# hidasib/GRU4Rec

Hardware: AMD Instinct MI355X
Metric: mini-batches/sec (gru4rec.py:661), RSC15-shaped batch=128 n_sample=2048 BPR-max (higher is better)
Workload: dtype f32

## Files before the change

gru4rec_amd/csrc/g4r_host_create.hpp:

```cpp

int g4r_device_count(void) {
    int n = 0;
    if (hipGetDeviceCount(&n) != hipSuccess) return 0;
    return n;
}
const char* g4r_last_error(void) { return g_err.c_str(); }
#ifndef G4R_HIPCC_VERSION
#define G4R_HIPCC_VERSION "unknown"
#endif
const char* g4r_version(void) { return "gru4rec_hip 0.4 (gfx950; hipcc " G4R_HIPCC_VERSION "; isa-audited)"; }
int g4r_sizeof_config(void) { return (int)sizeof(g4r_config); }

static int build_lean_args(g4r_model* m) {
    DevModel& d = m->dm;
    const StepKernels& k = m->kern;
    const int L = d.n_layers;
    std::vector<LeanV> av(L); std::vector<LeanH> ah(L); std::vector<LeanDa> aa(L); std::vector<LeanDy> ay(L);
    const bool constrained = d.embed_mode == G4R_EMBED_CONSTRAINED;
    bool any_layer = false;
    for (int l = 0; l < L; ++l) {
        if (k.fwd[l] != FWD_LEAN) continue;
        any_layer = true;
        LeanV& v = av[l]; memset(&v, 0, sizeof(v));
        v.Wx = d.dense_p + d.offWx[l]; v.Wrz = d.dense_p + d.offWrz[l]; v.Bh = d.dense_p + d.offBh[l];
// ... 56 lines not shown
        const size_t nslot = cdiv((long long)d.R * 16 * sizeof(int), (long long)sizeof(DenseTile));
        if (dalloc(m, &m->d_tiles16, tiles.size() + nslot) || dalloc(m, &m->d_leanU, (size_t)1)) return -1;
        d.own_pos = m->sw.owner_scan_in_update ? nullptr : (int*)(m->d_tiles16 + tiles.size());
        m->h_leanU.own_on = d.own_pos ? 1 : 0;
        HIPCHK(hipMemcpyAsync(m->d_tiles16, tiles.data(), tiles.size() * sizeof(DenseTile), hipMemcpyHostToDevice, m->stream));
        HIPCHK(hipStreamSynchronize(m->stream));
    }
    HIPCHK(hipStreamSynchronize(m->stream));
    return 0;
}

static KernelSwitches read_switches(const g4r_config& cfg) {
    KernelSwitches w;
    w.no_lean = getenv("G4R_NO_LEAN") != nullptr; w.no_mt = getenv("G4R_NO_MT") != nullptr; w.no_bmt = getenv("G4R_NO_BMT") != nullptr;
    w.no_merge = getenv("G4R_NO_MERGE") != nullptr; w.owner_scan_in_update = env_int("G4R_OWNER_SCAN", 0) != 0;
    w.allow_lean_update = env_int("G4R_LEAN_UPDATE", 1) != 0; w.defer = env_int("G4R_DEFER", cfg.defer_updates) != 0;
    w.p2_geo = env_int("G4R_P2_GEO", -1); w.ba_geo = env_int("G4R_BA_GEO", -1);
    w.wide2 = env_int("G4R_WIDE2", -1); w.p1_ks = env_int("G4R_P1_KS", 128); w.bb_ks = env_int("G4R_BB_KS", 0);
    const char* skip = getenv("G4R_SKIP_KN");
    w.skip_kn = skip ? strtoull(skip, nullptr, 0) : 0ull;
    return w;
}

int g4r_create(const g4r_config* cfg, g4r_model** out) {
    if (!cfg || !out) return fail("null argument");
    if (cfg->n_layers < 1 || cfg->n_layers > G4R_MAX_LAYERS) return fail("n_layers out of range");
    if (cfg->batch_size < 1 || cfg->n_items < 1) return fail("batch_size / n_items must be positive");
    for (int l = 0; l < cfg->n_layers; ++l)
        if (cfg->layers[l] % 4 != 0 || cfg->layers[l] < 4 || cfg->layers[l] > 1024)
            return fail("layer sizes must be multiples of 4 in [4, 1024]");
// ... 259 lines not shown
```

gru4rec_amd/csrc/g4r_host_debug.hpp:

```cpp
int g4r_get_debug(g4r_model* m, const char* name, float* host, int64_t count) {
    if (!m || !name || !host) return fail("null argument");
    HIPCHK(hipSetDevice(m->cfg.device));
    DevModel& d = m->dm;
    const StepKernels& k = m->kern;
    std::string s(name);
    const float* p = nullptr; int64_t n = 0;
    int l = 0;
    if (!s.empty() && isdigit((unsigned char)s.back())) { l = s.back() - '0'; s.pop_back(); }
    if (l >= d.n_layers) return fail("layer out of range");
    const int64_t bd = (int64_t)d.B * d.D[l];
    if (s == "scores") { p = d.Sc; n = (int64_t)d.B * d.ldSc; }
    else if (s == "dSx") { p = d.dSx + (size_t)((m->gstep - 1) & d.defer_mask) * (size_t)d.dSx_stride; n = (int64_t)d.B * d.Ein; }
    else if (s == "dSy") { p = d.dSy + (size_t)((m->gstep - 1) & d.defer_mask) * (size_t)d.dSy_stride; n = (int64_t)d.ldSc * d.Dtop; }
    else if (s == "dSBy") { p = d.dSBy + (size_t)((m->gstep - 1) & d.defer_mask) * (size_t)d.dSBy_stride; n = d.ldSc; }
    else if (s == "defer_stats") {
        if (count < 4) return fail("count");
        double rows = 0, bias = 0;
        if (m->defer_on) {
            std::vector<unsigned> st(2048);
            HIPCHK(hipStreamSynchronize(m->stream));
            HIPCHK(hipMemcpy(st.data(), d.dstat, st.size() * sizeof(unsigned), hipMemcpyDeviceToHost));
            for (size_t i = 0; i < st.size(); i += 2) { rows += st[i]; bias += st[i + 1]; }
        }
        host[0] = (float)rows; host[1] = (float)bias; host[2] = m->defer_on ? 1.f : 0.f; host[3] = (float)(d.defer_mask + 1);
// ... 36 lines not shown
        for (int l = 0; l < d.n_layers; ++l) mk |= k.fwd[l] == FWD_LEAN ? 1 << l : 0;
        host[0] = (float)mk; host[1] = k.score_fwd == SF_LEAN ? 1.f : 0.f; host[2] = k.score_bwd == SB_LEAN ? 1.f : 0.f;
        host[3] = k.update == UP_LEAN ? 1.f : 0.f;
        return 0;
    }
    else if (s == "kernels") {
        const int ML = G4R_MAX_LAYERS;
        const int tail[] = {k.score_fwd, k.loss_spec, k.loss_long, k.loss_quads, k.score_bwd, k.kch, k.ksplit, k.bmt_slabs, k.update, k.chunks, k.wide_dense, k.finish_rows};
        if (count < 4 * ML + 12) return fail("count");
        for (int i = 0; i < 4 * ML + 12; ++i) host[i] = i < 4 * ML ? 0.f : (float)tail[i - 4 * ML];
        for (int l = 0; l < d.n_layers; ++l) {
            host[l] = (float)k.fwd[l]; host[ML + l] = (float)k.bwd[l]; host[2 * ML + l] = (float)(k.p2_deep[l] + 2 * k.ba_deep[l]); host[3 * ML + l] = (float)k.wg[l].use;
        }
        return 0;
    }
    else if (s == "n_cu") { if (count < 1) return fail("count"); host[0] = (float)m->n_cu; return 0; }
    else if (s == "ksplit") { if (count < 1) return fail("count"); host[0] = (float)d.ksplit; return 0; }
    else if (s == "dev_syncs") { if (count < 1) return fail("count"); host[0] = (float)m->n_dev_syncs; return 0; }
    else if (s == "dense_count") { if (count < 1) return fail("count"); host[0] = (float)d.dense_count; return 0; }
    else if (s == "occ_score_tile") {
        if (count < 1) return fail("count");
        int nb = 0;
        for (size_t lds = SMEM_SF2; lds >= SMEM_SF2 - 2048; lds -= 512) {
            HIPCHK(hipOccupancyMaxActiveBlocksPerMultiprocessor(&nb, (const void*)k_score_fwd_t2, GT_NTH, lds));
            fprintf(stderr, "[g4r] k_score_fwd_t2 dynamic LDS %zu -> %d workgroups per CU\n", lds, nb);
        }
        host[0] = (float)nb;
        return 0;
    }
    else if (s == "graph_mode") {
// ... 132 lines not shown
```

gru4rec_amd/csrc/g4r_host_model.hpp:

```cpp
static thread_local std::string g_err;
static int fail(const std::string& s) { g_err = s; return -1; }
void g4r_set_error(const char* fmt, ...) {
    char buf[1024];
    va_list ap;
    va_start(ap, fmt);
    vsnprintf(buf, sizeof(buf), fmt, ap);
    va_end(ap);
    g_err = buf;
}
#define HIPCHK(x)                                                                                        \
    do {                                                                                                 \
        hipError_t e_ = (x);                                                                             \
        if (e_ != hipSuccess)                                                                            \
            return fail(std::string(#x) + ": " + hipGetErrorString(e_) + " @" + std::to_string(__LINE__)); \
    } while (0)
#define NCCLCHK(x)                                                                                         \
    do {                                                                                                   \
        ncclResult_t e_ = (x);                                                                             \
        if (e_ != ncclSuccess)                                                                             \
            return fail(std::string(#x) + ": " + ncclGetErrorString(e_) + " @" + std::to_string(__LINE__)); \
    } while (0)

enum { KN_GRU_P1 = 0, KN_GRU_P2, KN_SCORE_FWD, KN_LOSS, KN_SCORE_BWD, KN_BWD_PRE, KN_BWD_A, KN_BWD_B, KN_DENSE, KN_ALLREDUCE,
       KN_DENSE_APPLY, KN_SPARSE, KN_UPDATE, KN_BWD_FUSED, KN_FWD_FUSED, KN_GATE, KN_FLUSH, KN_SCAN, KN_FINISH, KN_GRU_V, KN_GRU_H, KN_GRU_DA, KN_GRU_DY, KN_COUNT };
static const char* KN_NAMES[KN_COUNT] = {"k_gru_p1", "k_gru_p2", "k_score_fwd", "k_loss_rows", "k_score_bwd", "k_gru_bwd_pre",
                                         "k_gru_bwd_a", "k_gru_bwd_b", "k_dense_grad", "rccl_allreduce", "k_dense_apply",
                                         "k_sparse_update", "k_update", "k_gru_bwd", "k_gru_fwd", "k_gru_gate", "k_sparse_flush", "k_defer_scan", "k_finish_rows", "k_gru_v", "k_gru_h", "k_gru_da", "k_gru_dy"};

struct EvRec { int kn; hipEvent_t a, b; };

struct KernelSwitches {
    bool no_lean = false;
    bool no_mt = false, no_bmt = false;
    bool no_merge = false;
    bool allow_lean_update = true;
    bool owner_scan_in_update = false;
    bool defer = false;
    int p2_geo = -1, ba_geo = -1;
    int wide2 = -1, p1_ks = 128, bb_ks = 0;
    unsigned long long skip_kn = 0;
};
enum GruFwdKind { FWD_LEAN = 0 , FWD_FUSED = 1 , FWD_P1S = 2 ,
                  FWD_P1_N64 = 3, FWD_P1_N32 = 4 };
enum GruBwdKind { BWD_LEAN = 0 , BWD_FUSED = 1 , BWD_ONEHOT = 2, BWD_BW = 3, BWD_B = 4 };
enum ScoreFwdKind { SF_LEAN = 0 , SF_MT = 1 , SF_T3 = 2, SF_T2 = 3, SF_K64 = 4, SF_K128 = 5  };
enum ScoreBwdKind { SB_LEAN = 0 , SB_BMT = 1 , SB_BWD2 = 2 , SB_W = 3, SB_N = 4  };
enum UpdateKind { UP_LEAN = 0 , UP_MERGED = 1 , UP_SPLIT = 2 };
struct WideGeo { int use = 0, ny = 1, nh = 1, kys = 0, khs = 0, bbn = 1, bbk = 0; };
struct StepKernels {
    int fwd[G4R_MAX_LAYERS], bwd[G4R_MAX_LAYERS];
    int p2_deep[G4R_MAX_LAYERS], ba_deep[G4R_MAX_LAYERS];
    WideGeo wg[G4R_MAX_LAYERS];
    int score_fwd;
    int loss_spec, loss_long, loss_quads;
    int score_bwd;
    int kch, ksplit;
    int bmt_slabs;
    int nblkA, nblkB, ndtA, ndtB, nrtB;
    int update;
    int chunks;
    int wide_dense;
    int finish_rows;
};

struct g4r_model {
    g4r_config cfg;
    DevModel dm;
    DevModel* d_dm = nullptr;
    int n_cu = 256;
    KernelSwitches sw;
// ... 234 lines not shown
    const bool lean_s = !sw.no_lean && Dt <= LN_MAXD && Dt % 4 == 0 && !wide && !dma && B < 65536 && d.ldSc < 65536;
    k.score_fwd = lean_s ? SF_LEAN : mt ? SF_MT : dma ? SF_T3 : (wide && Dt % T2_BK == 0) ? SF_T2 : wide ? SF_K64 : SF_K128;
    k.loss_spec = (d.final_act == G4R_ACT_ELU && d.loss == G4R_LOSS_BPR_MAX) ? 1 : (d.final_act == G4R_ACT_SOFTMAX && d.loss == G4R_LOSS_XE) ? 2
                : (d.final_act == G4R_ACT_ELU && d.loss == G4R_LOSS_TOP1_MAX) ? 3 : 0;
    k.loss_long = (size_t)(2 * d.ldSc + 18 * LOSS_NW) * sizeof(float) > (size_t)(156 * 1024);
    k.loss_quads = d.ldSc >= 4 * LOSS_T;
    const bool bwd2 = wide && Dt % 64 == 0;
    const bool top_tiles = k.bwd[top] != BWD_LEAN && k.bwd[top] != BWD_FUSED;
    if (!sw.no_bmt && bwd2 && top_tiles && Dt % 128 == 0 && Dt <= 512 && d.ldSc % BMT_WA == 0 && d.ldSc <= 0xFFFF && B <= 0xFFFF) {
        const int ntA = d.ldSc / BMT_WA * (Dt / 32), den = cdiv(B, 64) * (Dt / 128), ks = ntA / den;
        if (ntA % den == 0 && ntA % 8 == 0 && ntA <= n_cu && ntA * 8 >= n_cu * 7 && BMT_WA % (Dt / 32) == 0 && 4 * (BMT_WA / (Dt / 32)) <= 256 &&
            ks >= 2 && ks <= 24 && d.ldSc % ks == 0 && (d.ldSc / ks) % 32 == 0 && d.ldSc / ks <= 2048)
            k.bmt_slabs = ks;
    }
    k.score_bwd = (lean_s && B <= 128) ? SB_LEAN : k.bmt_slabs ? SB_BMT : bwd2 ? SB_BWD2 : wide ? SB_W : SB_N;
    const int slabs_target = top_tiles ? 17 : 9;
    k.kch = GT_BK * std::max(1, (cdiv(d.ldSc, GT_BK) + slabs_target / 2) / slabs_target);
    if (k.score_bwd == SB_LEAN) k.kch = 128;
    else if (k.score_bwd == SB_BMT) k.kch = d.ldSc / k.bmt_slabs;
    else if (k.score_bwd == SB_BWD2) {
        const int ndt = Dt / 64, nrt = cdiv(B, 64), nA = cdiv(d.ldSc, 64) * ndt;
        double best = 2.0;
        for (int ks = 12; ks <= 24; ++ks) {
            const int kch = (cdiv(d.ldSc, ks) + 7) & ~7;
            if (cdiv(d.ldSc, kch) != ks) continue;
            const double rounds = (double)(nA + ks * nrt * ndt) / n_cu;
            const double waste = (std::ceil(rounds) - rounds) / std::ceil(rounds) + 1e-3 * std::abs(ks - 17);
            if (waste < best) { best = waste; k.kch = kch; }
        }
    }
// ... 20 lines not shown
```

gru4rec_amd/csrc/g4r_host_step.hpp:

```cpp
static int launch_step(g4r_model* m, std::vector<EvRec>* recs, int part = 0) {
    DevModel& d = m->dm;
    const StepKernels& k = m->kern;
    const int L = d.n_layers, B = d.B;
    hipStream_t s = m->stream;
    GruFwdPredict nopa = {};
    size_t evi = 0;
    hipEvent_t cur_a = nullptr, cur_b = nullptr;
    static const bool trace = getenv("G4R_TRACE") != nullptr;
    int trace_kn = -1;
    auto begin = [&](int kn) {
        trace_kn = kn;
        if (trace) { fprintf(stderr, "[g4r] launch %s\n", KN_NAMES[kn]); fflush(stderr); }
        if (!recs) return;
        while (m->evs.size() < evi + 2) { hipEvent_t e; (void)hipEventCreate(&e); m->evs.push_back(e); }
        EvRec r = {kn, m->evs[evi], m->evs[evi + 1]};
        evi += 2;
        cur_a = r.a; cur_b = r.b;
        recs->push_back(r);
    };
    auto end = [&]() {
        if (trace) {
            hipError_t e = hipStreamSynchronize(s);
            fprintf(stderr, "[g4r] done   %s: %s\n", KN_NAMES[trace_kn], hipGetErrorString(e));
            fflush(stderr);
        }
    };
#define LK(kern, grid, block, smem, strm, ...)                                                             \
    do {                                                                                                  \
        if (m->sw.skip_kn && trace_kn >= 0 && ((m->sw.skip_kn >> trace_kn) & 1ull)) break;                \
        if (recs) hipExtLaunchKernelGGL(kern, grid, block, smem, strm, cur_a, cur_b, 0, __VA_ARGS__);     \
        else hipLaunchKernelGGL(kern, grid, block, smem, strm, __VA_ARGS__);                              \
    } while (0)
    const DevModel* dmp = (const DevModel*)m->d_dm;
    StepState* stp = (StepState*)d.st;
    const bool merged = k.update != UP_SPLIT && !(recs && m->profile_split);
    if (part != 2) {
    for (int l = 0; l < L; ++l) {
        if (k.fwd[l] == FWD_LEAN) {
            const int ntd = cdiv(d.D[l], 16), nrb = cdiv(B, 16);
            begin(KN_GRU_V);
            {
                const LeanV& v = m->h_leanV[l];
                const unsigned dims = (unsigned)d.D[l] | ((unsigned)d.IN[l] << 16);
#define G4R_LK_V(L0_, DR_) LK((k_gru_v<L0_, DR_>), dim3(ntd, nrb, 3), dim3(512), 0, s, (const LeanV*)(m->d_leanV + l), (StepState*)v.st, (const int*)v.cur_in, \
                              (const float*)v.Wx, (const float*)v.Wrz, (const float*)v.H0, (const float*)v.H1, dims, (unsigned)B)
                if (l > 0) G4R_LK_V(false, false); else if (d.drop_e > 0.f) G4R_LK_V(true, true); else G4R_LK_V(true, false);
#undef G4R_LK_V
            }
            end();
            begin(KN_GRU_H);
// ... 58 lines not shown
        do {                                                                                                                   \
            if (k.loss_spec == 1) LK((k_loss_rows<L, 1, V>), gloss, dim3(LOSS_T), m->smem_loss, s, dmp, stp);        \
            else if (k.loss_spec == 2) LK((k_loss_rows<L, 2, V>), gloss, dim3(LOSS_T), m->smem_loss, s, dmp, stp);   \
            else if (k.loss_spec == 3) LK((k_loss_rows<L, 3, V>), gloss, dim3(LOSS_T), m->smem_loss, s, dmp, stp);   \
            else LK((k_loss_rows<L, 0, V>), gloss, dim3(LOSS_T), m->smem_loss, s, dmp, stp);                         \
        } while (0)
        if (k.loss_long) G4R_LK_LOSS(true, 4);
        else { if (k.loss_quads) G4R_LK_LOSS(false, 4); else G4R_LK_LOSS(false, 1); }
#undef G4R_LK_LOSS
    }
    end();
    begin(KN_SCORE_BWD);
    switch (k.score_bwd) {
    case SB_LEAN: {
        const LeanB& q = m->h_leanB;
        LK(k_score_b, dim3(q.nA + d.ksplit * q.nrb * q.ndb), dim3(512), 0, s, (const LeanB*)m->d_leanB, (const int*)(d.cur_in + 2 * B), (const int*)d.cur_col,
           (const float*)d.Sc, (const float*)d.hd[L - 1], (const float*)d.Wy, (float*)d.accWy, (unsigned)d.Dtop | ((unsigned)B << 16), (unsigned)d.N | ((unsigned)d.ldSc << 16));
        break;
    }
    case SB_BMT: {
        const int ntile = d.ldSc / BMT_WA * (d.Dtop / 32);
        LK(k_score_bmt, dim3(2 * ntile), dim3(256), SMEM_BMT, s, (const float*)d.Sc, (const float*)d.hd[L - 1], (const float*)d.Wy, (const int*)d.col_item,
           (const int*)(d.cur_in + 2 * B), (const float*)d.zrow, dmp, (unsigned)d.Dtop | ((unsigned)(d.Dtop / 32) << 16), (unsigned)d.N | ((unsigned)d.ldSc << 16),
           (unsigned)B | ((unsigned)d.kch << 16), (unsigned)cdiv(B, 64) | ((unsigned)(d.Dtop / 128) << 16));
        break;
    }
    case SB_BWD2: {
        const int ndt = d.Dtop / 64, nrt = cdiv(B, 64);
        int nA = cdiv(d.ldSc, 64) * ndt, nB = d.ksplit * nrt * ndt, nC = cdiv(d.ldSc, 64);
        LK(k_score_bwd2, dim3(nA + nB + nC), dim3(GT_NTH), (size_t)(4 * 64 * 16) * sizeof(float) + (size_t)std::max(d.kch, 64) * sizeof(int), s, dmp, stp, nA, nB, ndt, nrt);
        break;
    }
// ... 2 lines not shown
    }
    end();
    for (int l = L - 1; l >= 0; --l) {
        if (k.bwd[l] == BWD_LEAN) {
            const int nrb = cdiv(B, 16);
            begin(KN_GRU_DA);
            {
                const LeanDa& q = m->h_leanDa[l];
                LK(k_gru_da, dim3(cdiv(d.D[l], 16), nrb), dim3(128), 0, s, (const LeanDa*)(m->d_leanDa + l), (const int*)(d.cur_in + 2 * B), (const float*)q.dsrc,
                   (const float*)q.Wh, (const float*)q.z, (const float*)q.c, (const float*)q.H0, (const float*)q.H1, (unsigned)d.D[l] | ((unsigned)q.ks << 16), (unsigned)B);
            }
            end();
            begin(KN_GRU_DY);
            {
                const LeanDy& y = m->h_leanDy[l];
                LK(k_gru_dy, dim3(cdiv(d.IN[l], 16), nrb), dim3(1024), 0, s, (const LeanDy*)(m->d_leanDy + l), (const int*)(d.cur_in + 2 * B), (const int*)y.occ_idx,
                   (const float*)y.dV, (const float*)y.drp, (const float*)y.Wx, (const float*)y.r, (unsigned)d.D[l] | ((unsigned)d.IN[l] << 16), (unsigned)B);
            }
            end();
            continue;
        }
        if (k.bwd[l] == BWD_FUSED) {
            begin(KN_BWD_FUSED);
            LK(k_gru_bwd_fused, dim3(cdiv(d.IN[l], 32), cdiv(B, BF_ROWS)), dim3(512), smem_bwd_fused(d.D[l]), s, dmp, stp, l);
            end();
            continue;
        }
        begin(KN_BWD_PRE);
        LK(k_gru_bwd_pre, dim3(cdiv((long long)B * d.D[l], 256)), dim3(256), 0, s, dmp, stp, l);
        end();
// ... 438 lines not shown
```

gru4rec_amd/csrc/g4r_lean_kernels.cuh:

```cuda
#pragma once

#define LN_MAXD 128

__device__ __forceinline__ float ldu(const GAS float* base, unsigned boff) { return *(const GAS float*)((const GAS char*)base + boff); }
__device__ __forceinline__ int ldu_i(const GAS int* base, unsigned boff) { return *(const GAS int*)((const GAS char*)base + boff); }
__device__ __forceinline__ float4 ldu4(const GAS float* base, unsigned boff) { return *(const GAS float4*)((const GAS char*)base + boff); }
__device__ __forceinline__ void stu(GAS float* base, unsigned boff, float v) { *(GAS float*)((GAS char*)base + boff) = v; }
__device__ __forceinline__ void stu4(GAS float* base, unsigned boff, float4 v) { *(GAS float4*)((GAS char*)base + boff) = v; }

#if defined(G4R_CLK_TRACE)
#define LCLK_INIT(dbgp, slot) GAS long long* clk_ = ((dbgp) && blockIdx.x == 1 && blockIdx.y == 1 && blockIdx.z == 0 && threadIdx.x == 0) ? (dbgp) + (slot) : nullptr
#define LCLK(i) do { if (clk_) clk_[i] = wall_clock64(); } while (0)
#define LCLK_USE(x) do { if (clk_ && (x) == 123.456f) clk_[15] = 0; } while (0)
#define LSPAN_BEGIN(tilep, base) GAS long long* span_ = ((tilep) && threadIdx.x == 0) ? (tilep) + 8 * (size_t)((base) + (blockIdx.z * gridDim.y + blockIdx.y) * gridDim.x + blockIdx.x) : nullptr; \
    if (span_) span_[0] = wall_clock64()
#define LSPAN_END() do { if (span_) span_[1] = wall_clock64(); } while (0)
#else
#define LCLK_INIT(dbgp, slot)
#define LCLK(i)
#define LCLK_USE(x)
#define LSPAN_BEGIN(tilep, base)
#define LSPAN_END()
#endif

struct LeanV {
    GP(const float) Wx; GP(const float) Wrz; GP(const float) Bh; GP(const float) H0; GP(const float) H1;
    GP(const float) ysrc;
    GP(const int) cur_in;
    GP(float) Vc; GP(float) r; GP(float) Hr; GP(float) z; GP(float) yin0;
    GP(int) occ_idx; GP(int) occ_fl;
    GP(StepState) st;
    unsigned long long seed;
    int B, D, IN, R, first, pub_fl;
    float drop_e;
    int n_items;
    GP(long long) dbg; GP(long long) dbgtile;
};
// ... 334 lines not shown
    for (int q = 0; q < 4; ++q) acc[q] = mfma16(bq[q].w, da[3], acc[q]);
    LCLK_USE(acc[0][0]); LCLK(5);
    if ((int)row < M) {
        const unsigned ob = j * ps + 4 * (row * D + 4 * lg);
#pragma unroll
        for (int q = 0; q < 4; ++q) {
            const unsigned n = 16 * (4 * wid + q) + 4 * lg;
            if (n < D) stu4(a.drp, ob + 64 * (4 * wid + q), make_float4(acc[q][0], acc[q][1], acc[q][2], acc[q][3]));
        }
    }
    LCLK(6);
    LSPAN_END();
}

#define LN_PL 8
__global__ __launch_bounds__(1024) void k_gru_dy(const LeanDy* __restrict__ ap, const int* meta_, const int* occ_idx_, const float* dV_, const float* drp_,
                                                 const float* Wx_, const float* r_, unsigned dims, unsigned B) {
    __shared__ float sJ[4 * 16 * 64];
    const unsigned tid = threadIdx.x, lane = tid & 63, li = lane & 15, lg = lane >> 4;
    const unsigned wid = __builtin_amdgcn_readfirstlane(tid >> 6);
    const unsigned D = dims & 0xFFFFu, IN = dims >> 16, Dq = D >> 2;
    const unsigned m0 = blockIdx.y * 16, row = m0 + li, rowB = min(row, B - 1);
    const unsigned ncol = 16 * blockIdx.x + li, nc = min(ncol, IN - 1);
    const unsigned rowe = m0 + 4 * lg + (wid & 3);
    const GAS float* Wx = (const GAS float*)Wx_;
#if defined(G4R_CLK_TRACE)
    const long long tk0 = wall_clock64();
    GAS long long* ck = nullptr;
#define DYCK(i) do { if (ck) ck[i] = wall_clock64(); } while (0)
#else
#define DYCK(i)
#endif
    f32x4 acc;
// ... 82 lines not shown
        acc1 = mfma16(s.w, b0.w, acc1);
        acc = acc0 + acc1;
#if defined(G4R_CLK_TRACE)
        if (ck) { if (acc[0] == 123.4f) ck[7] = 0; ck[3] = wall_clock64(); }
#endif
    }
    const int M = sx.M;
    if ((int)m0 >= M) return;
#pragma unroll
    for (int rg = 0; rg < 4; ++rg) sJ[(rg * 16 + wid) * 64 + lane] = acc[rg];
    __syncthreads();
    if (wid >= 4) return;
    const LeanDy a = *ap;
    LCLK_INIT(a.dbg, 48); LCLK(6);
    LSPAN_BEGIN(a.dbgtile, 1500);
    float v = 0.f;
#pragma unroll
    for (int w = 0; w < 16; ++w) v += sJ[(wid * 16 + w) * 64 + lane];
    if (ncol >= IN || (int)rowe >= M) return;
    const unsigned o = 4 * (rowe * IN + ncol);
    if (a.layer0) {
        if (a.drop_e > 0.f) v *= drop_mult(a.seed, sx.g, G4R_STREAM_DROP_EMBED, rowe, ncol, 1.0f - a.drop_e);
        const float an = a2 + G4R_MUT_ACC(v * v);
        GAS float* dSx = a.dSx + (size_t)(sx.g & (unsigned)a.defer_mask) * (size_t)a.dSx_stride;
        stu(dSx, o, a.generic ? v : G4R_MUT_STEP(a.lr * v * frsq(an + G4R_EPS_ADAGRAD)));
        if (!a.generic && cnt2 == 1 && itm >= 0) a.accT[(size_t)itm * IN + ncol] = an;
        else stu(a.dAx, o, an);
    } else {
        stu(a.dylo, o, v);
    }
    LCLK(7);
    LSPAN_END();
}

template <bool LOGQ>
__global__ __launch_bounds__(256) void k_score_s(const LeanS* __restrict__ ap, const int* meta_, const int* cur_col_, const float* hd_, const float* Wy_,
                                                 const float* By_, float* Sc_, unsigned dimsA, unsigned dimsB) {
    __shared__ f32x4 sJ[4 * 4 * 64];
    const unsigned tid = threadIdx.x, lane = tid & 63, li = lane & 15, lg = lane >> 4;
    const unsigned wid = __builtin_amdgcn_readfirstlane(tid >> 6);
    const unsigned D = dimsA & 0xFFFFu, B = dimsA >> 16, N = dimsB & 0xFFFFu, ldSc = dimsB >> 16, Dq = D >> 2;
    const unsigned n0 = blockIdx.x * 32, m0 = blockIdx.y * 32;
    const GAS int* cur_col = (const GAS int*)cur_col_;
    const unsigned nA = n0 + li, nB = n0 + 16 + li;
    int it0 = ldu_i(cur_col, 4 * min(nA, ldSc - 1)), it1 = ldu_i(cur_col, 4 * min(nB, ldSc - 1));
    const int4 mt = ldi4((const GAS int*)meta_);
    const unsigned Q0 = 8 * wid + lg, Q1 = Q0 + 4;
// ... 65 lines not shown
    if (ne >= N) return;
    const unsigned r0 = m0 + 16 * (wid >> 1) + 4 * lg;
    GAS float* Sc = (GAS float*)Sc_;
    float o[4];
#pragma unroll
    for (int rg = 0; rg < 4; ++rg) { o[rg] = v[rg] + bias; lean_keep(o[rg]); }
#pragma unroll
    for (int rg = 0; rg < 4; ++rg)
        if ((int)(r0 + rg) < M) stu(Sc, 4 * ((r0 + rg) * ldSc + ne), o[rg]);
    LCLK(5);
    LSPAN_END();
}
template __global__ void k_score_s<false>(const LeanS*, const int*, const int*, const float*, const float*, const float*, float*, unsigned, unsigned);
template __global__ void k_score_s<true>(const LeanS*, const int*, const int*, const float*, const float*, const float*, float*, unsigned, unsigned);

__global__ __launch_bounds__(512) void k_score_b(const LeanB* __restrict__ ap, const int* meta_, const int* cur_col_, const float* Sc_, const float* hd_,
                                                 const float* Wy_, float* accWy_, unsigned dimsA, unsigned dimsB) {
    __shared__ f32x4 sJ[4 * 8 * 64];
    const unsigned tid = threadIdx.x, lane = tid & 63, li = lane & 15, lg = lane >> 4;
    const unsigned wid = __builtin_amdgcn_readfirstlane(tid >> 6);
    const unsigned D = dimsA & 0xFFFFu, B = dimsA >> 16, N = dimsB & 0xFFFFu, ldSc = dimsB >> 16;
    const GAS int* cur_col = (const GAS int*)cur_col_;
    const GAS float *Sc = (const GAS float*)Sc_, *hd = (const GAS float*)hd_;
    const int4 mt = ldi4((const GAS int*)meta_);
    const LeanB a = *ap;
    LSPAN_BEGIN(a.dbgtile, 2048);
    f32x4 acc[4];
#pragma unroll
    for (int c = 0; c < 4; ++c) acc[c] = (f32x4){0.f, 0.f, 0.f, 0.f};
    if (blockIdx.x < (unsigned)a.nA) {
        const unsigned nt = blockIdx.x / (unsigned)a.ndh, dh_ = blockIdx.x - nt * (unsigned)a.ndh;
        const unsigned n0 = 16 * nt, d0 = 64 * dh_;
        const unsigned n = n0 + li, nc = min(n, ldSc - 1);
        const unsigned d4 = d0 + 16 * lg + 4 * (wid & 3);
        const int item = ldu_i(cur_col, 4 * nc);
        float4 av[4];
        float bv[4];
        const unsigned da = d0 + 4 * li;
        const unsigned dac = min(da, D - 4);
#pragma unroll
        for (int s_ = 0; s_ < 4; ++s_) {
            const unsigned b = min(16 * wid + 4 * s_ + lg, B - 1);
            av[s_] = ldu4(hd, 4 * (b * D + dac));
            bv[s_] = ldu(Sc, 4 * (b * ldSc + nc));
        }
        lean_pin(a.accBy, a.occ_fl);
        const bool iok = item >= 0 && n < N;
        const unsigned ic = (unsigned)max(item, 0);
        float4 acc4 = ld4((const GAS float*)accWy_ + (size_t)ic * D + min(d4, D - 4));
        const float accb = a.accBy[ic];
        const int cnt = a.occ_fl[4 * (size_t)ic + 2];
        if (d4 >= D) acc4 = make_float4(accb, 0.f, 0.f, 0.f);
        __builtin_amdgcn_sched_barrier(0);
        const LeanState sx = lean_state(mt);
        const int M = sx.M;
#pragma unroll
        for (int s_ = 0; s_ < 4; ++s_) {
            const unsigned b = 16 * wid + 4 * s_ + lg;
            const bool bok = (int)b < M;
            float4 h4 = av[s_];
            const float hx[4] = {h4.x, h4.y, h4.z, h4.w};
            float hv[4];
#pragma unroll
            for (int c = 0; c < 4; ++c) hv[c] = (da + c < D) ? hx[c] : ((da + c == D) ? 1.f : 0.f);
            const float dsv = (bok && n < ldSc) ? bv[s_] : 0.f;
#pragma unroll
            for (int c = 0; c < 4; ++c) acc[c] = mfma16(hv[c], dsv, acc[c]);
        }
#pragma unroll
        for (int rg = 0; rg < 4; ++rg) sJ[(rg * 8 + wid) * 64 + lane] = (f32x4){acc[0][rg], acc[1][rg], acc[2][rg], acc[3][rg]};
        __syncthreads();
        if (wid >= 4) return;
        f32x4 g4 = sJ[(wid * 8 + 0) * 64 + lane];
#pragma unroll
        for (int w = 1; w < 8; ++w) g4 += sJ[(wid * 8 + w) * 64 + lane];
        if (n >= N || d4 > D) return;
        const float gg[4] = {g4[0], g4[1], g4[2], g4[3]}, a0[4] = {acc4.x, acc4.y, acc4.z, acc4.w};
        float st[4], an[4];
        const bool generic = a.generic != 0;
#pragma unroll
        for (int c = 0; c < 4; ++c) {
            an[c] = a0[c] + G4R_MUT_ACC(gg[c] * gg[c]);
            st[c] = iok ? G4R_MUT_ROW(n, G4R_MUT_STEP(a.lr * gg[c] * frsq(an[c] + G4R_EPS_ADAGRAD))) : 0.f;
            if (generic) st[c] = iok ? gg[c] : 0.f;
        }
        const bool single = !generic && iok && cnt == 1;
        const size_t slot = (size_t)(sx.g & (unsigned)a.defer_mask);
        if (d4 < D) {
            st4(a.dSy + slot * (size_t)a.dSy_stride + (size_t)n * D + d4, make_float4(st[0], st[1], st[2], st[3]));
            if (single) st4((GAS float*)accWy_ + (size_t)ic * D + d4, make_float4(an[0], an[1], an[2], an[3]));
            else st4(a.dAy + (size_t)n * D + d4, make_float4(an[0], an[1], an[2], an[3]));
        } else {
            (a.dSBy + slot * (size_t)a.dSBy_stride)[n] = st[0];
            if (single) a.accBy[ic] = an[0]; else a.dABy[n] = an[0];
        }
        LSPAN_END();
        return;
    }
    {
        const unsigned w_ = blockIdx.x - (unsigned)a.nA;
        const unsigned per = (unsigned)(a.nrb * a.ndb);
        const unsigned kc = w_ / per, rem = w_ - kc * per, rb = rem / (unsigned)a.ndb, db = rem - rb * (unsigned)a.ndb;
        const unsigned b0 = 16 * rb, d0 = 64 * db;
        const unsigned nk = 128 * kc + 16 * wid + 4 * lg;
        const unsigned nkc = min(nk, ldSc - 4);
        const int4 it4 = ldi4(cur_col + nkc);
        float4 ds4 = ldu4(Sc, 4 * (min(b0 + li, B - 1) * ldSc + nkc));
        const unsigned dq = d0 + 4 * li, dqc = min(dq, D - 4);
        const GAS float* Wy = (const GAS float*)Wy_;
        const int its[4] = {it4.x, it4.y, it4.z, it4.w};
        float4 wv[4];
#pragma unroll
        for (int u = 0; u < 4; ++u) wv[u] = ld4(Wy + (size_t)max(its[u], 0) * D + dqc);
        __builtin_amdgcn_sched_barrier(0);
        const LeanState sx = lean_state(mt);
        const int M = sx.M;
        if ((int)b0 >= M) return;
        const float dsx[4] = {ds4.x, ds4.y, ds4.z, ds4.w};
        const bool bok = (int)(b0 + li) < M;
#pragma unroll
        for (int u = 0; u < 4; ++u) {
            const bool kok = nk + u < ldSc && nk == nkc && its[u] >= 0 && dq < D;
            const float av_ = bok ? dsx[u] : 0.f;
            const float4 w4 = kok ? wv[u] : make_float4(0.f, 0.f, 0.f, 0.f);
            acc[0] = mfma16(av_, w4.x, acc[0]);
            acc[1] = mfma16(av_, w4.y, acc[1]);
            acc[2] = mfma16(av_, w4.z, acc[2]);
            acc[3] = mfma16(av_, w4.w, acc[3]);
        }
#pragma unroll
        for (int rg = 0; rg < 4; ++rg) sJ[(rg * 8 + wid) * 64 + lane] = (f32x4){acc[0][rg], acc[1][rg], acc[2][rg], acc[3][rg]};
        __syncthreads();
        if (wid >= 4) return;
        f32x4 v = sJ[(wid * 8 + 0) * 64 + lane];
#pragma unroll
        for (int w = 1; w < 8; ++w) v += sJ[(wid * 8 + w) * 64 + lane];
        const unsigned b = b0 + 4 * lg + (wid & 3);
        if ((int)b < M && dq < D) st4(a.dhpart + ((size_t)kc * B + b) * D + dq, make_float4(v[0], v[1], v[2], v[3]));
        LSPAN_END();
    }
}

template <bool MOM>
__device__ __forceinline__ void lean_rows_update(const LeanU& a, const GAS int* occ_idx, GAS int* occ_fl, const GAS float* dSx, const GAS float* dSy,
                                                 const GAS float* dSBy, const GAS int* opos_t, unsigned k, unsigned R, unsigned B) {
    const unsigned lane = threadIdx.x & 63;
    const bool tableE = k < B && !a.constrained;
    const unsigned W = tableE ? (unsigned)a.wE : (unsigned)a.wY, nc4 = W >> 2;
    const unsigned c4 = min(lane, nc4 - 1);
    const bool lok = lane < nc4;
    const unsigned kc = min(k, R - 1);
    int item = ldu_i(occ_idx, 4 * kc);
    const int opos = ldu_i(opos_t, 4 * (16 * kc + min(lane, 15u)));
    const GAS float* srow = (kc < B) ? dSx + (size_t)kc * W : dSy + (size_t)(kc - B) * W;
    const float4 sk = ld4(srow + 4 * c4);
// ... 275 lines not shown
```

Baseline: 25820.

## Move score-backward Wy-gradient tiles into the top-layer GRU dy kernel launch

Splits the lean score-backward kernel into two templated roles. When the top layer also uses the lean backward path, the Wy/By gradient and Adagrad tiles (role A) are taken out of k_score_b and run as extra 1024-thread workgroups of a new k_gru_dy_a launch, two tiles per workgroup, beside the dy tiles. The goal is a smaller score-backward grid and a shorter critical path, with the independent role-A work hidden under the dy kernel. In exchange the fused kernel uses more shared memory per workgroup, and the role-A writes now happen later in the step. The switch is on by default and can be turned off with G4R_SCORE_B_SPLIT.

```diff
diff --git a/gru4rec_amd/csrc/g4r_host_create.hpp b/gru4rec_amd/csrc/g4r_host_create.hpp
--- a/gru4rec_amd/csrc/g4r_host_create.hpp
+++ b/gru4rec_amd/csrc/g4r_host_create.hpp
@@ -94,6 +94,7 @@
     KernelSwitches w;
     w.no_lean = getenv("G4R_NO_LEAN") != nullptr; w.no_mt = getenv("G4R_NO_MT") != nullptr; w.no_bmt = getenv("G4R_NO_BMT") != nullptr;
     w.no_merge = getenv("G4R_NO_MERGE") != nullptr; w.owner_scan_in_update = env_int("G4R_OWNER_SCAN", 0) != 0;
+    w.score_b_split = env_int("G4R_SCORE_B_SPLIT", 1) != 0;
     w.allow_lean_update = env_int("G4R_LEAN_UPDATE", 1) != 0; w.defer = env_int("G4R_DEFER", cfg.defer_updates) != 0;
     w.p2_geo = env_int("G4R_P2_GEO", -1); w.ba_geo = env_int("G4R_BA_GEO", -1);
     w.wide2 = env_int("G4R_WIDE2", -1); w.p1_ks = env_int("G4R_P1_KS", 128); w.bb_ks = env_int("G4R_BB_KS", 0);
diff --git a/gru4rec_amd/csrc/g4r_host_debug.hpp b/gru4rec_amd/csrc/g4r_host_debug.hpp
--- a/gru4rec_amd/csrc/g4r_host_debug.hpp
+++ b/gru4rec_amd/csrc/g4r_host_debug.hpp
@@ -74,6 +74,7 @@
         }
         return 0;
     }
+    else if (s == "score_b_split") { if (count < 1) return fail("count"); host[0] = (float)k.score_a_host; return 0; }
     else if (s == "n_cu") { if (count < 1) return fail("count"); host[0] = (float)m->n_cu; return 0; }
     else if (s == "ksplit") { if (count < 1) return fail("count"); host[0] = (float)d.ksplit; return 0; }
     else if (s == "dev_syncs") { if (count < 1) return fail("count"); host[0] = (float)m->n_dev_syncs; return 0; }
diff --git a/gru4rec_amd/csrc/g4r_host_model.hpp b/gru4rec_amd/csrc/g4r_host_model.hpp
--- a/gru4rec_amd/csrc/g4r_host_model.hpp
+++ b/gru4rec_amd/csrc/g4r_host_model.hpp
@@ -34,6 +34,7 @@
     bool no_mt = false, no_bmt = false;
     bool no_merge = false;
     bool allow_lean_update = true;
+    bool score_b_split = true;
     bool owner_scan_in_update = false;
     bool defer = false;
     int p2_geo = -1, ba_geo = -1;
@@ -54,6 +55,7 @@
     int score_fwd;
     int loss_spec, loss_long, loss_quads;
     int score_bwd;
+    int score_a_host;
     int kch, ksplit;
     int bmt_slabs;
     int nblkA, nblkB, ndtA, ndtB, nrtB;
@@ -318,6 +320,7 @@
             k.bmt_slabs = ks;
     }
     k.score_bwd = (lean_s && B <= 128) ? SB_LEAN : k.bmt_slabs ? SB_BMT : bwd2 ? SB_BWD2 : wide ? SB_W : SB_N;
+    k.score_a_host = (sw.score_b_split && k.score_bwd == SB_LEAN && k.bwd[top] == BWD_LEAN) ? 1 : 0;
     const int slabs_target = top_tiles ? 17 : 9;
     k.kch = GT_BK * std::max(1, (cdiv(d.ldSc, GT_BK) + slabs_target / 2) / slabs_target);
     if (k.score_bwd == SB_LEAN) k.kch = 128;
diff --git a/gru4rec_amd/csrc/g4r_host_step.hpp b/gru4rec_amd/csrc/g4r_host_step.hpp
--- a/gru4rec_amd/csrc/g4r_host_step.hpp
+++ b/gru4rec_amd/csrc/g4r_host_step.hpp
@@ -34,6 +34,7 @@
     const DevModel* dmp = (const DevModel*)m->d_dm;
     StepState* stp = (StepState*)d.st;
     const bool merged = k.update != UP_SPLIT && !(recs && m->profile_split);
+    const bool a_hosted = k.score_a_host && !recs;
     if (part != 2) {
     for (int l = 0; l < L; ++l) {
         if (k.fwd[l] == FWD_LEAN) {
@@ -122,8 +123,11 @@
     switch (k.score_bwd) {
     case SB_LEAN: {
         const LeanB& q = m->h_leanB;
-        LK(k_score_b, dim3(q.nA + d.ksplit * q.nrb * q.ndb), dim3(512), 0, s, (const LeanB*)m->d_leanB, (const int*)(d.cur_in + 2 * B), (const int*)d.cur_col,
-           (const float*)d.Sc, (const float*)d.hd[L - 1], (const float*)d.Wy, (float*)d.accWy, (unsigned)d.Dtop | ((unsigned)B << 16), (unsigned)d.N | ((unsigned)d.ldSc << 16));
+#define G4R_LK_SB(RA, NWG) LK(k_score_b<RA>, dim3(NWG), dim3(512), 0, s, (const LeanB*)m->d_leanB, (const int*)(d.cur_in + 2 * B), (const int*)d.cur_col,   \
+           (const float*)d.Sc, (const float*)d.hd[L - 1], (const float*)d.Wy, (float*)d.accWy, (unsigned)d.Dtop | ((unsigned)B << 16), (unsigned)d.N | ((unsigned)d.ldSc << 16))
+        if (a_hosted) G4R_LK_SB(false, d.ksplit * q.nrb * q.ndb);
+        else G4R_LK_SB(true, q.nA + d.ksplit * q.nrb * q.ndb);
+#undef G4R_LK_SB
         break;
     }
     case SB_BMT: {
@@ -156,6 +160,14 @@
             begin(KN_GRU_DY);
             {
                 const LeanDy& y = m->h_leanDy[l];
+                if (a_hosted && l == L - 1) {
+                    const LeanB& q = m->h_leanB;
+                    const int gx = cdiv(d.IN[l], 16);
+                    LK(k_gru_dy_a, dim3(gx, nrb + cdiv(cdiv(q.nA, 2), gx)), dim3(1024), 0, s, (const LeanDy*)(m->d_leanDy + l), (const int*)(d.cur_in + 2 * B),
+                       (const int*)y.occ_idx, (const float*)y.dV, (const float*)y.drp, (const float*)y.Wx, (const float*)y.r, (unsigned)d.D[l] | ((unsigned)d.IN[l] << 16),
+                       (unsigned)B, (const LeanB*)m->d_leanB, (const int*)d.cur_col, (const float*)d.Sc, (const float*)d.hd[L - 1], (float*)d.accWy,
+                       (unsigned)d.Dtop | ((unsigned)B << 16), (unsigned)d.N | ((unsigned)d.ldSc << 16), (unsigned)q.nA | ((unsigned)q.ndh << 16));
+                } else
                 LK(k_gru_dy, dim3(cdiv(d.IN[l], 16), nrb), dim3(1024), 0, s, (const LeanDy*)(m->d_leanDy + l), (const int*)(d.cur_in + 2 * B), (const int*)y.occ_idx,
                    (const float*)y.dV, (const float*)y.drp, (const float*)y.Wx, (const float*)y.r, (unsigned)d.D[l] | ((unsigned)d.IN[l] << 16), (unsigned)B);
             }
diff --git a/gru4rec_amd/csrc/g4r_lean_kernels.cuh b/gru4rec_amd/csrc/g4r_lean_kernels.cuh
--- a/gru4rec_amd/csrc/g4r_lean_kernels.cuh
+++ b/gru4rec_amd/csrc/g4r_lean_kernels.cuh
@@ -15,12 +15,15 @@
 #define LSPAN_BEGIN(tilep, base) GAS long long* span_ = ((tilep) && threadIdx.x == 0) ? (tilep) + 8 * (size_t)((base) + (blockIdx.z * gridDim.y + blockIdx.y) * gridDim.x + blockIdx.x) : nullptr; \
     if (span_) span_[0] = wall_clock64()
 #define LSPAN_END() do { if (span_) span_[1] = wall_clock64(); } while (0)
+#define LSPAN_BEGIN_AT(tilep, idx, lead) GAS long long* span_ = ((tilep) && (lead)) ? (tilep) + 8 * (size_t)(idx) : nullptr; \
+    if (span_) span_[0] = wall_clock64()
 #else
 #define LCLK_INIT(dbgp, slot)
 #define LCLK(i)
 #define LCLK_USE(x)
 #define LSPAN_BEGIN(tilep, base)
 #define LSPAN_END()
+#define LSPAN_BEGIN_AT(tilep, idx, lead)
 #endif
 
 struct LeanV {
@@ -385,9 +388,8 @@
 }
 
 #define LN_PL 8
-__global__ __launch_bounds__(1024) void k_gru_dy(const LeanDy* __restrict__ ap, const int* meta_, const int* occ_idx_, const float* dV_, const float* drp_,
-                                                 const float* Wx_, const float* r_, unsigned dims, unsigned B) {
-    __shared__ float sJ[4 * 16 * 64];
+__device__ __forceinline__ void gru_dy_tile(const LeanDy* __restrict__ ap, const int* meta_, const int* occ_idx_, const float* dV_, const float* drp_,
+                                            const float* Wx_, const float* r_, const unsigned dims, const unsigned B, float* sJ) {
     const unsigned tid = threadIdx.x, lane = tid & 63, li = lane & 15, lg = lane >> 4;
     const unsigned wid = __builtin_amdgcn_readfirstlane(tid >> 6);
     const unsigned D = dims & 0xFFFFu, IN = dims >> 16, Dq = D >> 2;
@@ -500,6 +502,9 @@
     const LeanDy a = *ap;
     LCLK_INIT(a.dbg, 48); LCLK(6);
     LSPAN_BEGIN(a.dbgtile, 1500);
+#if defined(G4R_CLK_TRACE)
+    if (span_) { span_[2] = span_[0]; span_[0] = tk0; }
+#endif
     float v = 0.f;
 #pragma unroll
     for (int w = 0; w < 16; ++w) v += sJ[(wid * 16 + w) * 64 + lane];
@@ -517,6 +522,11 @@
     }
     LCLK(7);
     LSPAN_END();
+}
+__global__ __launch_bounds__(1024) void k_gru_dy(const LeanDy* __restrict__ ap, const int* meta_, const int* occ_idx_, const float* dV_, const float* drp_,
+                                                 const float* Wx_, const float* r_, unsigned dims, unsigned B) {
+    __shared__ float sJ[4 * 16 * 64];
+    gru_dy_tile(ap, meta_, occ_idx_, dV_, drp_, Wx_, r_, dims, B, sJ);
 }
 
 template <bool LOGQ>
@@ -612,131 +622,168 @@
 template __global__ void k_score_s<false>(const LeanS*, const int*, const int*, const float*, const float*, const float*, float*, unsigned, unsigned);
 template __global__ void k_score_s<true>(const LeanS*, const int*, const int*, const float*, const float*, const float*, float*, unsigned, unsigned);
 
+__device__ __forceinline__ void score_b_role_a(const LeanB& a, const int4 mt, const GAS int* cur_col, const GAS float* Sc, const GAS float* hd, float* accWy_,
+                                               const unsigned D, const unsigned B, const unsigned N, const unsigned ldSc, const unsigned t, const unsigned ndh,
+                                               const unsigned wid, const unsigned lane, f32x4* sJ, const bool live, const bool lead) {
+    const unsigned li = lane & 15, lg = lane >> 4;
+    LSPAN_BEGIN_AT(a.dbgtile, 2048 + t, lead && live);
+    f32x4 acc[4];
+#pragma unroll
+    for (int c = 0; c < 4; ++c) acc[c] = (f32x4){0.f, 0.f, 0.f, 0.f};
+    const unsigned nt = t / ndh, dh_ = t - nt * ndh;
+    const unsigned n0 = 16 * nt, d0 = 64 * dh_;
+    const unsigned n = n0 + li, nc = min(n, ldSc - 1);
+    const unsigned d4 = d0 + 16 * lg + 4 * (wid & 3);
+    const int item = ldu_i(cur_col, 4 * nc);
+    float4 av[4];
+    float bv[4];
+    const unsigned da = d0 + 4 * li;
+    const unsigned dac = min(da, D - 4);
+#pragma unroll
+    for (int s_ = 0; s_ < 4; ++s_) {
+        const unsigned b = min(16 * wid + 4 * s_ + lg, B - 1);
+        av[s_] = ldu4(hd, 4 * (b * D + dac));
+        bv[s_] = ldu(Sc, 4 * (b * ldSc + nc));
+    }
+    lean_pin(a.accBy, a.occ_fl);
+    const bool iok = item >= 0 && n < N;
+    const unsigned ic = (unsigned)max(item, 0);
+    float4 acc4 = ld4((const GAS float*)accWy_ + (size_t)ic * D + min(d4, D - 4));
+    const float accb = a.accBy[ic];
+    const int cnt = a.occ_fl[4 * (size_t)ic + 2];
+    if (d4 >= D) acc4 = make_float4(accb, 0.f, 0.f, 0.f);
+    __builtin_amdgcn_sched_barrier(0);
+    const LeanState sx = lean_state(mt);
+    const int M = sx.M;
+#pragma unroll
+    for (int s_ = 0; s_ < 4; ++s_) {
+        const unsigned b = 16 * wid + 4 * s_ + lg;
+        const bool bok = (int)b < M;
+        float4 h4 = av[s_];
+        const float hx[4] = {h4.x, h4.y, h4.z, h4.w};
+        float hv[4];
+#pragma unroll
+        for (int c = 0; c < 4; ++c) hv[c] = (da + c < D) ? hx[c] : ((da + c == D) ? 1.f : 0.f);
+        const float dsv = (bok && n < ldSc) ? bv[s_] : 0.f;
+#pragma unroll
+        for (int c = 0; c < 4; ++c) acc[c] = mfma16(hv[c], dsv, acc[c]);
+    }
+#pragma unroll
+    for (int rg = 0; rg < 4; ++rg) sJ[(rg * 8 + wid) * 64 + lane] = (f32x4){acc[0][rg], acc[1][rg], acc[2][rg], acc[3][rg]};
+    __syncthreads();
+    if (wid >= 4 || !live) return;
+    f32x4 g4 = sJ[(wid * 8 + 0) * 64 + lane];
+#pragma unroll
+    for (int w = 1; w < 8; ++w) g4 += sJ[(wid * 8 + w) * 64 + lane];
+    if (n >= N || d4 > D) return;
+    const float gg[4] = {g4[0], g4[1], g4[2], g4[3]}, a0[4] = {acc4.x, acc4.y, acc4.z, acc4.w};
+    float st[4], an[4];
+    const bool generic = a.generic != 0;
+#pragma unroll
+    for (int c = 0; c < 4; ++c) {
+        an[c] = a0[c] + G4R_MUT_ACC(gg[c] * gg[c]);
+        st[c] = iok ? G4R_MUT_ROW(n, G4R_MUT_STEP(a.lr * gg[c] * frsq(an[c] + G4R_EPS_ADAGRAD))) : 0.f;
+        if (generic) st[c] = iok ? gg[c] : 0.f;
+    }
+    const bool single = !generic && iok && cnt == 1;
+    const size_t slot = (size_t)(sx.g & (unsigned)a.defer_mask);
+    if (d4 < D) {
+        st4(a.dSy + slot * (size_t)a.dSy_stride + (size_t)n * D + d4, make_float4(st[0], st[1], st[2], st[3]));
+        if (single) st4((GAS float*)accWy_ + (size_t)ic * D + d4, make_float4(an[0], an[1], an[2], an[3]));
+        else st4(a.dAy + (size_t)n * D + d4, make_float4(an[0], an[1], an[2], an[3]));
+    } else {
+        (a.dSBy + slot * (size_t)a.dSBy_stride)[n] = st[0];
+        if (single) a.accBy[ic] = an[0]; else a.dABy[n] = an[0];
+    }
+    LSPAN_END();
+}
+
+__device__ __forceinline__ void score_b_role_b(const LeanB& a, const int4 mt, const GAS int* cur_col, const GAS float* Sc, const float* Wy_,
+                                               const unsigned D, const unsigned B, const unsigned ldSc, const unsigned w_,
+                                               const unsigned wid, const unsigned lane, f32x4* sJ) {
+    const unsigned li = lane & 15, lg = lane >> 4;
+    LSPAN_BEGIN_AT(a.dbgtile, 2048 + (unsigned)a.nA + w_, threadIdx.x == 0);
+    f32x4 acc[4];
+#pragma unroll
+    for (int c = 0; c < 4; ++c) acc[c] = (f32x4){0.f, 0.f, 0.f, 0.f};
+    const unsigned per = (unsigned)(a.nrb * a.ndb);
+    const unsigned kc = w_ / per, rem = w_ - kc * per, rb = rem / (unsigned)a.ndb, db = rem - rb * (unsigned)a.ndb;
+    const unsigned b0 = 16 * rb, d0 = 64 * db;
+    const unsigned nk = 128 * kc + 16 * wid + 4 * lg;
+    const unsigned nkc = min(nk, ldSc - 4);
+    const int4 it4 = ldi4(cur_col + nkc);
+    float4 ds4 = ldu4(Sc, 4 * (min(b0 + li, B - 1) * ldSc + nkc));
+    const unsigned dq = d0 + 4 * li, dqc = min(dq, D - 4);
+    const GAS float* Wy = (const GAS float*)Wy_;
+    const int its[4] = {it4.x, it4.y, it4.z, it4.w};
+    float4 wv[4];
+#pragma unroll
+    for (int u = 0; u < 4; ++u) wv[u] = ld4(Wy + (size_t)max(its[u], 0) * D + dqc);
+    __builtin_amdgcn_sched_barrier(0);
+    const LeanState sx = lean_state(mt);
+    const int M = sx.M;
+    if ((int)b0 >= M) return;
+    const float dsx[4] = {ds4.x, ds4.y, ds4.z, ds4.w};
+    const bool bok = (int)(b0 + li) < M;
+#pragma unroll
+    for (int u = 0; u < 4; ++u) {
+        const bool kok = nk + u < ldSc && nk == nkc && its[u] >= 0 && dq < D;
+        const float av_ = bok ? dsx[u] : 0.f;
+        const float4 w4 = kok ? wv[u] : make_float4(0.f, 0.f, 0.f, 0.f);
+        acc[0] = mfma16(av_, w4.x, acc[0]);
+        acc[1] = mfma16(av_, w4.y, acc[1]);
+        acc[2] = mfma16(av_, w4.z, acc[2]);
+        acc[3] = mfma16(av_, w4.w, acc[3]);
+    }
+#pragma unroll
+    for (int rg = 0; rg < 4; ++rg) sJ[(rg * 8 + wid) * 64 + lane] = (f32x4){acc[0][rg], acc[1][rg], acc[2][rg], acc[3][rg]};
+    __syncthreads();
+    if (wid >= 4) return;
+    f32x4 v = sJ[(wid * 8 + 0) * 64 + lane];
+#pragma unroll
+    for (int w = 1; w < 8; ++w) v += sJ[(wid * 8 + w) * 64 + lane];
+    const unsigned b = b0 + 4 * lg + (wid & 3);
+    if ((int)b < M && dq < D) st4(a.dhpart + ((size_t)kc * B + b) * D + dq, make_float4(v[0], v[1], v[2], v[3]));
+    LSPAN_END();
+}
+
+template <bool ROLE_A>
 __global__ __launch_bounds__(512) void k_score_b(const LeanB* __restrict__ ap, const int* meta_, const int* cur_col_, const float* Sc_, const float* hd_,
                                                  const float* Wy_, float* accWy_, unsigned dimsA, unsigned dimsB) {
     __shared__ f32x4 sJ[4 * 8 * 64];
-    const unsigned tid = threadIdx.x, lane = tid & 63, li = lane & 15, lg = lane >> 4;
+    const unsigned tid = threadIdx.x, lane = tid & 63;
     const unsigned wid = __builtin_amdgcn_readfirstlane(tid >> 6);
     const unsigned D = dimsA & 0xFFFFu, B = dimsA >> 16, N = dimsB & 0xFFFFu, ldSc = dimsB >> 16;
     const GAS int* cur_col = (const GAS int*)cur_col_;
     const GAS float *Sc = (const GAS float*)Sc_, *hd = (const GAS float*)hd_;
     const int4 mt = ldi4((const GAS int*)meta_);
     const LeanB a = *ap;
-    LSPAN_BEGIN(a.dbgtile, 2048);
-    f32x4 acc[4];
-#pragma unroll
-    for (int c = 0; c < 4; ++c) acc[c] = (f32x4){0.f, 0.f, 0.f, 0.f};
-    if (blockIdx.x < (unsigned)a.nA) {
-        const unsigned nt = blockIdx.x / (unsigned)a.ndh, dh_ = blockIdx.x - nt * (unsigned)a.ndh;
-        const unsigned n0 = 16 * nt, d0 = 64 * dh_;
-        const unsigned n = n0 + li, nc = min(n, ldSc - 1);
-        const unsigned d4 = d0 + 16 * lg + 4 * (wid & 3);
-        const int item = ldu_i(cur_col, 4 * nc);
-        float4 av[4];
-        float bv[4];
-        const unsigned da = d0 + 4 * li;
-        const unsigned dac = min(da, D - 4);
-#pragma unroll
-        for (int s_ = 0; s_ < 4; ++s_) {
-            const unsigned b = min(16 * wid + 4 * s_ + lg, B - 1);
-            av[s_] = ldu4(hd, 4 * (b * D + dac));
-            bv[s_] = ldu(Sc, 4 * (b * ldSc + nc));
-        }
-        lean_pin(a.accBy, a.occ_fl);
-        const bool iok = item >= 0 && n < N;
-        const unsigned ic = (unsigned)max(item, 0);
-        float4 acc4 = ld4((const GAS float*)accWy_ + (size_t)ic * D + min(d4, D - 4));
-        const float accb = a.accBy[ic];
-        const int cnt = a.occ_fl[4 * (size_t)ic + 2];
-        if (d4 >= D) acc4 = make_float4(accb, 0.f, 0.f, 0.f);
-        __builtin_amdgcn_sched_barrier(0);
-        const LeanState sx = lean_state(mt);
-        const int M = sx.M;
-#pragma unroll
-        for (int s_ = 0; s_ < 4; ++s_) {
-            const unsigned b = 16 * wid + 4 * s_ + lg;
-            const bool bok = (int)b < M;
-            float4 h4 = av[s_];
-            const float hx[4] = {h4.x, h4.y, h4.z, h4.w};
-            float hv[4];
-#pragma unroll
-            for (int c = 0; c < 4; ++c) hv[c] = (da + c < D) ? hx[c] : ((da + c == D) ? 1.f : 0.f);
-            const float dsv = (bok && n < ldSc) ? bv[s_] : 0.f;
-#pragma unroll
-            for (int c = 0; c < 4; ++c) acc[c] = mfma16(hv[c], dsv, acc[c]);
-        }
-#pragma unroll
-        for (int rg = 0; rg < 4; ++rg) sJ[(rg * 8 + wid) * 64 + lane] = (f32x4){acc[0][rg], acc[1][rg], acc[2][rg], acc[3][rg]};
-        __syncthreads();
-        if (wid >= 4) return;
-        f32x4 g4 = sJ[(wid * 8 + 0) * 64 + lane];
-#pragma unroll
-        for (int w = 1; w < 8; ++w) g4 += sJ[(wid * 8 + w) * 64 + lane];
-        if (n >= N || d4 > D) return;
-        const float gg[4] = {g4[0], g4[1], g4[2], g4[3]}, a0[4] = {acc4.x, acc4.y, acc4.z, acc4.w};
-        float st[4], an[4];
-        const bool generic = a.generic != 0;
-#pragma unroll
-        for (int c = 0; c < 4; ++c) {
-            an[c] = a0[c] + G4R_MUT_ACC(gg[c] * gg[c]);
-            st[c] = iok ? G4R_MUT_ROW(n, G4R_MUT_STEP(a.lr * gg[c] * frsq(an[c] + G4R_EPS_ADAGRAD))) : 0.f;
-            if (generic) st[c] = iok ? gg[c] : 0.f;
-        }
-        const bool single = !generic && iok && cnt == 1;
-        const size_t slot = (size_t)(sx.g & (unsigned)a.defer_mask);
-        if (d4 < D) {
-            st4(a.dSy + slot * (size_t)a.dSy_stride + (size_t)n * D + d4, make_float4(st[0], st[1], st[2], st[3]));
-            if (single) st4((GAS float*)accWy_ + (size_t)ic * D + d4, make_float4(an[0], an[1], an[2], an[3]));
-            else st4(a.dAy + (size_t)n * D + d4, make_float4(an[0], an[1], an[2], an[3]));
-        } else {
-            (a.dSBy + slot * (size_t)a.dSBy_stride)[n] = st[0];
-            if (single) a.accBy[ic] = an[0]; else a.dABy[n] = an[0];
-        }
-        LSPAN_END();
-        return;
-    }
-    {
-        const unsigned w_ = blockIdx.x - (unsigned)a.nA;
-        const unsigned per = (unsigned)(a.nrb * a.ndb);
-        const unsigned kc = w_ / per, rem = w_ - kc * per, rb = rem / (unsigned)a.ndb, db = rem - rb * (unsigned)a.ndb;
-        const unsigned b0 = 16 * rb, d0 = 64 * db;
-        const unsigned nk = 128 * kc + 16 * wid + 4 * lg;
-        const unsigned nkc = min(nk, ldSc - 4);
-        const int4 it4 = ldi4(cur_col + nkc);
-        float4 ds4 = ldu4(Sc, 4 * (min(b0 + li, B - 1) * ldSc + nkc));
-        const unsigned dq = d0 + 4 * li, dqc = min(dq, D - 4);
-        const GAS float* Wy = (const GAS float*)Wy_;
-        const int its[4] = {it4.x, it4.y, it4.z, it4.w};
-        float4 wv[4];
-#pragma unroll
-        for (int u = 0; u < 4; ++u) wv[u] = ld4(Wy + (size_t)max(its[u], 0) * D + dqc);
-        __builtin_amdgcn_sched_barrier(0);
-        const LeanState sx = lean_state(mt);
-        const int M = sx.M;
-        if ((int)b0 >= M) return;
-        const float dsx[4] = {ds4.x, ds4.y, ds4.z, ds4.w};
-        const bool bok = (int)(b0 + li) < M;
-#pragma unroll
-        for (int u = 0; u < 4; ++u) {
-            const bool kok = nk + u < ldSc && nk == nkc && its[u] >= 0 && dq < D;
-            const float av_ = bok ? dsx[u] : 0.f;
-            const float4 w4 = kok ? wv[u] : make_float4(0.f, 0.f, 0.f, 0.f);
-            acc[0] = mfma16(av_, w4.x, acc[0]);
-            acc[1] = mfma16(av_, w4.y, acc[1]);
-            acc[2] = mfma16(av_, w4.z, acc[2]);
-            acc[3] = mfma16(av_, w4.w, acc[3]);
-        }
-#pragma unroll
-        for (int rg = 0; rg < 4; ++rg) sJ[(rg * 8 + wid) * 64 + lane] = (f32x4){acc[0][rg], acc[1][rg], acc[2][rg], acc[3][rg]};
-        __syncthreads();
-        if (wid >= 4) return;
-        f32x4 v = sJ[(wid * 8 + 0) * 64 + lane];
-#pragma unroll
-        for (int w = 1; w < 8; ++w) v += sJ[(wid * 8 + w) * 64 + lane];
-        const unsigned b = b0 + 4 * lg + (wid & 3);
-        if ((int)b < M && dq < D) st4(a.dhpart + ((size_t)kc * B + b) * D + dq, make_float4(v[0], v[1], v[2], v[3]));
-        LSPAN_END();
-    }
+    if (ROLE_A) {
+        if (blockIdx.x < (unsigned)a.nA) { score_b_role_a(a, mt, cur_col, Sc, hd, accWy_, D, B, N, ldSc, blockIdx.x, (unsigned)a.ndh, wid, lane, sJ, true, tid == 0); return; }
+        score_b_role_b(a, mt, cur_col, Sc, Wy_, D, B, ldSc, blockIdx.x - (unsigned)a.nA, wid, lane, sJ);
+    } else {
+        score_b_role_b(a, mt, cur_col, Sc, Wy_, D, B, ldSc, blockIdx.x, wid, lane, sJ);
+    }
+}
+template __global__ void k_score_b<true>(const LeanB*, const int*, const int*, const float*, const float*, const float*, float*, unsigned, unsigned);
+template __global__ void k_score_b<false>(const LeanB*, const int*, const int*, const float*, const float*, const float*, float*, unsigned, unsigned);
+
+__global__ __launch_bounds__(1024) void k_gru_dy_a(const LeanDy* __restrict__ ap, const int* meta_, const int* occ_idx_, const float* dV_, const float* drp_,
+                                                   const float* Wx_, const float* r_, unsigned dims, unsigned B, const LeanB* __restrict__ bp,
+                                                   const int* cur_col_, const float* Sc_, const float* hd_, float* accWy_, unsigned dimsA, unsigned dimsB, unsigned tilesA) {
+    __shared__ f32x4 sJ[2 * 4 * 8 * 64];
+    const unsigned nrb = (B + 15) >> 4;
+    if (blockIdx.y < nrb) { gru_dy_tile(ap, meta_, occ_idx_, dV_, drp_, Wx_, r_, dims, B, (float*)sJ); return; }
+    const unsigned tid = threadIdx.x, lane = tid & 63;
+    const unsigned wid = __builtin_amdgcn_readfirstlane(tid >> 6);
+    const unsigned nA = tilesA & 0xFFFFu, half = wid >> 3;
+    const unsigned t0 = 2 * ((blockIdx.y - nrb) * gridDim.x + blockIdx.x), t = t0 + half;
+    if (t0 >= nA) return;
+    const int4 mt = ldi4((const GAS int*)meta_);
+    const LeanB a = *bp;
+    const bool live = t < nA;
+    score_b_role_a(a, mt, (const GAS int*)cur_col_, (const GAS float*)Sc_, (const GAS float*)hd_, accWy_, dimsA & 0xFFFFu, dimsA >> 16, dimsB & 0xFFFFu,
+                   dimsB >> 16, live ? t : nA - 1, tilesA >> 16, wid & 7, lane, sJ + half * (4 * 8 * 64), live, (tid & 511) == 0);
 }
 
 template <bool MOM>
```

Result: faster. 26430, median of 6 (+2.4%).
